# yosungho/LineTR

Measured on AMD Instinct MI355X. Metric: line_descriptors_per_sec, higher is better.
Workload: dtype f32 in/out; GEMMs as 6 bf16-split MFMA products, fp32 accumulate (fp32-faithful); 1 GPU; cfg3: 64 pairs/GPU of 640x480, 200 lines/image -> 199 sub-lines x 21 tokens, d_model=256, seeded weights; pairs_per_gpu=64, collective=none

## Files before the change

### experiments/csrc/lt_x_net.h

```cpp
#pragma once
#include "lt_gemm_sk.h"
#include "lt_gemm_st.h"
#include "lt_gemm_ro.h"
#include "lt_gemm_chain.h"
#include "lt_mlp_fused.h"
#include "lt_attn_st.h"
#include "lt_pairnet_host.h"

namespace {

int x_gemm(LinetrHandle* h, hipStream_t st, SplitGemmArgs& sa, const GemmW& w, int groups, const NormSpec* fused_norm,
           double fl, double by, bool& done) {
  const GemmArgs& g = sa.g;
  if (h->precision == LINETR_PREC_BF16X6 && LT_XENV("LINETR_GEMM_RO") != nullptr && groups == 1 && g.N % 256 == 0 && g.K % 32 == 0 &&
      w.st && g.lda % 4 == 0 && g.ldy % 4 == 0 && (!g.A2 || (g.lda2 % 4 == 0 && g.K1 % 16 == 0)) && (!g.R || g.ldr % 4 == 0) &&
      g.act != ACT_DIST && cdiv(g.M, 128) * (g.N / 256) >= 140) {
    RoGemmArgs a;
    a.A1 = g.A; a.lda1 = g.lda; a.nk1 = (g.A2 ? g.K1 : g.K) / 16; a.A2 = g.A2; a.lda2 = g.lda2; a.nk2 = g.A2 ? (g.K - g.K1) / 16 : 0;
    a.Wst = w.st; a.bias = g.bias ? g.bias : h->zeros; a.R = g.R; a.ldr = g.ldr; a.Y = g.Y; a.ldy = g.ldy;
    a.M = g.M; a.N = g.N; a.act = g.act;
    if (fused_norm) { a.norm = fused_norm->mode; a.gamma = fused_norm->gamma; a.beta = fused_norm->beta; a.add2 = fused_norm->add2; a.ldadd2 = D; a.eps = fused_norm->eps; }
    done = true;
    ProfScope ps(h, st, "gemm_bf16x6_ro128x256", fl, by);
    return gemm_ro_launch(a, st);
// ... 141 lines not shown
    if (int e = sig_mlp_fused_launch<2, 1>(a, st)) return e;
  } else {
    a.W1sp = S.W1.s3; a.W2sp = S.W2p.s3;
    ProfScope ps(h, st, "sig_mlp_bf16x6", fl, by);
    if (int e = sig_mlp_fused_launch<3, 0>(a, st)) return e;
  }
  LT_LAUNCH_CHECK();
  return 0;
}

int sig_network_fused_mlp(LinetrHandle* h, hipStream_t st, const TokenStage& ts, const int32_t* h_cu, const int* cu_dev, int n_images,
                          int N, int max_n, float* d_line_desc, FwdWs& w) {
  const LinetrModelConfig& c = h->cfg;
  const double attn_fl = attn_flops(h_cu, n_images);
  const int64_t sig_bn_off = 4 * (int64_t)(c.enc_channels[0] + c.enc_channels[1] + c.enc_channels[2] + c.enc_channels[3]);
  const int attn_kernel = sig_attn_plan(h, n_images, N, max_n).attn;
  const bool fused_qkv_attn = !LT_XENV("LINETR_NO_FUSED_QKV_ATTN") && h->precision == LINETR_PREC_BF16X6 && max_n <= 256 &&
                              (int64_t)n_images * HEADS >= 128;
  float *z = w.zA, *zn = w.zB;
  int e;
  for (size_t l = 0;; ++l) {
    const SigLayer& S = h->sig[l];
    if (fused_qkv_attn && S.Wqkv.st) {
      if ((e = sig_qkv_attention(h, st, S, z, cu_dev, n_images, N, attn_fl, w.msgp))) return e;
    } else {
      if ((e = run_gemm(h, st, S.Wqkv, N, {z, D}, {w.qkv, 3 * D}, ACT_NONE))) return e;
      if ((e = sig_attention(h, st, attn_kernel, w.qkv, 3 * D, cu_dev, n_images, N, max_n, attn_fl, w.msgp))) return e;
    }
    if (l + 1 == h->sig.size()) break;
    if ((e = run_sig_mlp(h, st, z, w.msgp, S, zn, N))) return e;
    std::swap(z, zn);
  }
  const size_t l = h->sig.size() - 1;
  if ((e = run_gemm(h, st, h->sig[l].W1, N, {z, D, w.msgp, D, D}, {w.hid, 2 * D}, ts.bn ? ACT_NONE : ACT_RELU))) return e;
  if (ts.bn && (e = bn_train_layer(st, *ts.bn, w.hid, N, 2 * D, 2 * D, h->bn_g[8 + l], h->bn_b[8 + l], sig_bn_off + (int64_t)l * 4 * D))) return e;
  NormSpec l2; l2.mode = 2;
  return run_gemm_norm(h, st, h->Wfin2, N, {z, D, w.hid, 2 * D, D}, nullptr, zn, d_line_desc, l2);
}

int sig_network_st(LinetrHandle* h, hipStream_t st, FwdWs& w, const XWs& x, const int32_t* h_cu, const int* cu_dev, int n_images,
                   int N, int max_n, float* d_line_desc) {
  auto gemm = [&](const char* role, const unsigned char* A1, int K1, const unsigned char* A2, int K2, const GemmW& W,
                  const unsigned char* R, unsigned char* Yst, float* Y, int act) -> int {
    const int Nout = W.rows;
    StGemmArgs a;
    a.A1 = A1; a.nk1 = K1 / 16; a.A2 = A2; a.nk2 = A2 ? K2 / 16 : 0;
    a.W = W.st; a.bias = W.b ? W.b : h->zeros; a.R = R; a.Yst = Yst; a.Y = Y; a.ldy = D; a.M = N; a.N = Nout; a.act = act;
// ... 114 lines not shown
```

### include/linetr_hip.h

```cpp
#ifndef LINETR_HIP_H
#define LINETR_HIP_H

#include <stdint.h>

#ifdef __cplusplus
extern "C" {
#endif

#define LINETR_ABI_VERSION 6

enum {
  LINETR_OK = 0,
  LINETR_E_ARG = -1,
  LINETR_E_HIP = -2,
  LINETR_E_WEIGHTS = -3,
  LINETR_E_ASSERT = -4,
  LINETR_E_WORKSPACE = -5,
  LINETR_E_CAPACITY = -6
};

typedef struct LinetrHandle LinetrHandle;

typedef struct {
  int32_t d_model;
// ... 437 lines not shown
int linetr_debug_posenc(LinetrHandle* h, int32_t which, const float* d_in0, const float* d_in1, const float* d_in2,
                           int64_t rows, float* d_out, void* stream);

int linetr_debug_gemm(LinetrHandle* h, const float* d_A, int32_t lda, const float* d_W, const float* d_bias,
                      const float* d_residual, float* d_Y, int32_t ldy, int32_t M, int32_t N, int32_t K,
                      int32_t act, int32_t cache_weights, void* stream);

#define LINETR_GEMM_TILE_WS 100
typedef struct {
  const float* A;   int32_t lda;
  const float* A2;  int32_t lda2;  int32_t K1;
  const float* W;
  const float* bias;
  const float* R;
  float* Y;         int32_t ldy;
  int32_t M, N, K, act;
  int32_t groups;   int64_t gA, gY;
  int32_t norm;     const float* gamma;  const float* beta;  const float* add2;  float eps;
  int32_t via_row_norm;
  int32_t tile;
} LinetrGemmCase;
int linetr_debug_gemm_case(LinetrHandle* h, const LinetrGemmCase* c, int32_t* tile_used, void* stream);

int linetr_debug_sig_attention(LinetrHandle* h, int32_t kernel, int32_t layer, const float* d_in, int32_t ld_in,
                               const int32_t* h_cu_sub, int32_t n_images, float* d_msg, int32_t* kernel_used, void* stream);

int linetr_debug_tok_mlp(LinetrHandle* h, int32_t variant, const float* d_pnt, const float* d_score, int64_t rows_word,
                         const float* d_sublines, const float* d_resp, const float* d_angle, int64_t rows_line,
                         float* d_out_word, float* d_out_line, int32_t max_blocks, int32_t* variant_used, void* stream);

int64_t linetr_debug_bn_train_workspace_bytes(const LinetrHandle* h, int32_t which, int64_t rows);
int linetr_debug_bn_train(LinetrHandle* h, int32_t which, float* d_z, int64_t rows, int32_t C, int32_t ld, const float* d_gamma,
                          const float* d_beta, const float* d_in0, const float* d_in1, const float* d_in2, float* d_out,
                          float momentum, float* d_running, float* d_batch, float* d_affine, int32_t* nb_used, void* d_ws,
                          int64_t ws_bytes, void* stream);

int linetr_debug_cls_pool(LinetrHandle* h, int32_t kernel, const LinetrLineRec* d_recs, int32_t K, const int32_t* d_sub2line,
                          int32_t N, int32_t T, const float* d_cpnt, const float* d_a4, int64_t first_pad, int32_t n_images,
                          const float* d_map, int32_t dense_is_nhwc, int32_t Hc, int32_t Wc, int32_t align_corners,
                          const float* d_desc_dense, float* d_pooled, int32_t* kernel_used, void* stream);

int linetr_debug_match(LinetrHandle* h, int32_t P, const int32_t* dims, const float* d_desc0, const int64_t* off_n0,
                       const int32_t* d_s2l0, const float* d_desc1, const int64_t* off_n1, const int32_t* d_s2l1, float thr,
                       int32_t mutual, float* d_dk, const int64_t* off_dk, int32_t* d_match01, const int64_t* off_k0, void* d_ws,
                       int64_t ws_bytes, int32_t path, int32_t seg1_global, int32_t cache_dk, int32_t device_table,
                       int32_t* path_used, void* stream);
// ... 53 lines not shown
```

### linetr_amd/csrc/linetr_net.hip

```cpp
#include <algorithm>
#include <array>
#include <numeric>
#include <set>

#include "lt_handle.h"
#include "lt_gemm.h"
#include "lt_gemm_split.h"
#include "lt_gemm_split16.h"
#include "lt_st_image.h"
#include "lt_gemm_small.h"
#include "lt_model.h"
#include "lt_attn.h"
#include "lt_attn_fused.h"
#include "lt_gemm_ws.h"
#include "lt_tokmlp.h"
#include "lt_token.h"
#include "lt_bntrain.h"

using namespace lt;

namespace {

const char* gemm_class_name(int precision, int tile, const GemmArgs& g, int groups) {
  static const auto names = [] {
// ... 597 lines not shown
}

int cls_pooling(LinetrHandle* h, hipStream_t& st, const TokenStage& ts, int n_images, int N, int T, FwdWs& w) {
  if (int e = cls_pool_launch(h, st, cls_pool_plan(ts.cpnt != nullptr, N), ts, n_images, N, T, w.act[ENC_WORD][3], w.pooled)) return e;
  return value_projection(h, st, N, w.pooled, w.att);
}

int sentence(LinetrHandle* h, hipStream_t& st, int N, FwdWs& w) {
  const LinetrModelConfig& c = h->cfg;
  int e;
  {
    NormSpec ns; ns.mode = 1; ns.gamma = h->ln1g; ns.beta = h->ln1b; ns.eps = 1e-6f;
    if ((e = run_gemm_norm(h, st, h->Wfc, N, {w.att, D}, nullptr, w.fc, w.o, ns))) return e;
  }
  if ((e = run_gemm(h, st, h->Wf1, N, {w.o, D}, {w.f1, c.d_inner}, ACT_GELU))) return e;
  NormSpec ns; ns.mode = 1; ns.gamma = h->ln2g; ns.beta = h->ln2b; ns.add2 = w.lpos; ns.eps = 1e-6f;
  return run_gemm_norm(h, st, h->Wf2, N, {w.f1, c.d_inner}, w.o, w.f2, w.zA, ns);
}

enum { SIGK_F32 = 0, SIGK_SMALL = 1, SIGK_SPLIT4 = 2, SIGK_SPLIT8 = 3, SIGK_FUSED = 4 };
struct SigAttnPlan {
  int attn;
  bool fold_next, fused;
  int kernel() const { return fused ? SIGK_FUSED : attn; }
};
SigAttnPlan sig_attn_plan(const LinetrHandle* h, int n_images, int N, int max_n) {
  SigAttnPlan p;
  const bool small_attn = h->precision != LINETR_PREC_F32 && (int64_t)n_images * HEADS * cdiv(max_n, 256) < 64;
  p.attn = h->precision == LINETR_PREC_F32 ? SIGK_F32 : small_attn ? SIGK_SMALL : max_n <= 128 ? SIGK_SPLIT4 : SIGK_SPLIT8;
  p.fold_next = small_attn && N <= SIG_FOLD_MAX_ROWS && !LT_XENV("LINETR_NO_SIG_FOLD");
  p.fused = !p.fold_next && !LT_XENV("LINETR_NO_FUSED_QKV_ATTN") && h->precision == LINETR_PREC_BF16X6 && max_n <= 256 &&
            (int64_t)n_images * HEADS >= 128;
  return p;
}

int sig_plan_servable(const LinetrHandle* h, const SigAttnPlan& p, int N, int max_n) {
  if (p.attn < SIGK_F32 || p.attn > SIGK_SPLIT8) return fail(LINETR_E_ARG, "sig plan: attention kernel %d outside 0 .. 3", p.attn);
  if (h->precision == LINETR_PREC_F32 && (p.attn != SIGK_F32 || p.fused))
    return fail(LINETR_E_ARG, "sig plan: the f32 mode runs sig_attn_kernel (0) only");
  if (p.fold_next) {
    if (p.fused) return fail(LINETR_E_ARG, "sig plan: fold_next and the fused projection + attention exclude each other");
    if (p.attn != SIGK_SMALL) return fail(LINETR_E_ARG, "sig plan: fold_next leaves q/k/v at row stride 1024, which sig_attn_small (1) alone reads");
    if (N > SIG_FOLD_MAX_ROWS) return fail(LINETR_E_ARG, "sig plan: fold_next has buffers for up to %d sub-lines (got %d)", SIG_FOLD_MAX_ROWS, N);
  }
  if (p.fused) {
    if (h->precision != LINETR_PREC_BF16X6) return fail(LINETR_E_ARG, "sig plan: the fused projection + attention runs in bf16x6 mode only");
// ... 3 lines not shown
  }
  return LINETR_OK;
}

int sig_attention(LinetrHandle* h, hipStream_t st, int kernel, const float* qkv, int ldq, const int* cu_dev, int n_images, int N,
                  int max_n, double fl, float* msg) {
  if (kernel == SIGK_F32) {
    ProfScope ps(h, st, "sig_attn", fl, (double)N * D * 16);
    hipLaunchKernelGGL(sig_attn_kernel, dim3(n_images, HEADS, cdiv(max_n, ATT_QT)), dim3(256), 0, st, qkv, cu_dev, msg);
  } else {
    ProfScope ps(h, st, "sig_attn_bf16x6", fl, (double)N * D * 16);
    if (kernel == SIGK_SMALL)
      hipLaunchKernelGGL(sig_attn_small_kernel, dim3(n_images, HEADS, cdiv(max_n, 32)), dim3(256), 0, st, qkv, cu_dev, msg, ldq);
    else if (kernel == SIGK_SPLIT4)
      hipLaunchKernelGGL(sig_attn_split_kernel<4>, dim3(n_images, HEADS, cdiv(max_n, ATT_QT)), dim3(256), 0, st, qkv, cu_dev, msg);
    else
      hipLaunchKernelGGL(sig_attn_split_kernel<8>, dim3(n_images, HEADS, cdiv(max_n, 256)), dim3(512), 0, st, qkv, cu_dev, msg);
  }
  LT_LAUNCH_CHECK();
  return LINETR_OK;
}

int sig_qkv_attention(LinetrHandle* h, hipStream_t st, const SigLayer& S, const float* z, const int* cu_dev, int n_images, int N,
                      double attn_fl, float* msg) {
  LT_HIP(allow_dynamic_lds<sig_qkv_attn_kernel>(FQA_LDS));
  ProfScope ps(h, st, "sig_qkv_attn_bf16x6", 2.0 * N * 3.0 * D * D + attn_fl, (double)N * D * 8);
  hipLaunchKernelGGL(sig_qkv_attn_kernel, dim3(n_images, HEADS), dim3(512), FQA_LDS, st, z, S.Wqkv.st, S.Wqkv.b,
                     cu_dev, msg);
  LT_LAUNCH_CHECK();
  return LINETR_OK;
}

int sig_network(LinetrHandle* h, hipStream_t& st, const TokenStage& ts, const int32_t* h_cu, const int* cu_dev, int n_images, int N,
                float* d_line_desc, FwdWs& w, const SigAttnPlan* forced = nullptr) {
  const LinetrModelConfig& c = h->cfg;
  int max_n = 0;
  for (int i = 0; i < n_images; ++i) max_n = std::max(max_n, h_cu[i + 1] - h_cu[i]);
  int e;
  const double attn_fl = attn_flops(h_cu, n_images);
  const int64_t sig_bn_off = 4 * (int64_t)(c.enc_channels[0] + c.enc_channels[1] + c.enc_channels[2] + c.enc_channels[3]);
  const SigAttnPlan plan = forced ? *forced : sig_attn_plan(h, n_images, N, max_n);
  const bool fold_next = plan.fold_next, fused_qkv_attn = plan.fused;
  float *z = w.zA, *zn = w.zB;
  int ldz = D;
  float *zq = w.zqA, *zq_next = w.zqB;
  const float* qkv = w.qkv;
  int ldq = 3 * D;
  for (size_t l = 0; l < h->sig.size(); ++l) {
    const SigLayer& S = h->sig[l];
    if (fused_qkv_attn && S.Wqkv.st) {
      if ((e = sig_qkv_attention(h, st, S, z, cu_dev, n_images, N, attn_fl, w.msgp))) return e;
    } else {
      if (!fold_next || l == 0)
        if ((e = run_gemm(h, st, S.Wqkv, N, {z, ldz}, {w.qkv, 3 * D}, ACT_NONE))) return e;
      if ((e = sig_attention(h, st, plan.attn, qkv, ldq, cu_dev, n_images, N, max_n, attn_fl, w.msgp))) return e;
    }
    if ((e = run_gemm(h, st, S.W1, N, {z, ldz, w.msgp, D, D}, {w.hid, 2 * D}, ts.bn ? ACT_NONE : ACT_RELU))) return e;
    if (ts.bn && (e = bn_train_layer(st, *ts.bn, w.hid, N, 2 * D, 2 * D, h->bn_g[8 + l], h->bn_b[8 + l], sig_bn_off + (int64_t)l * 4 * D))) return e;
    if (l + 1 == h->sig.size()) break;
    if (fold_next) {
      if ((e = run_gemm(h, st, S.Wnext, N, {z, ldz, w.hid, 2 * D, D}, {zq, 4 * D}, ACT_NONE))) return e;
      z = zq; ldz = 4 * D; qkv = zq + D; ldq = 4 * D;
      std::swap(zq, zq_next);
    } else {
      if ((e = run_gemm(h, st, S.W2, N, {w.hid, 2 * D}, {zn, D}, ACT_NONE, z))) return e;
      std::swap(z, zn);
    }
    if (w.tap)
      LT_HIP(hipMemcpy2DAsync(w.tap + (int64_t)l * N * D, D * sizeof(float), z, ldz * sizeof(float), D * sizeof(float), N,
                              hipMemcpyDeviceToDevice, st));
    if ((e = pipe_boundary(ts.pipe, CUT_SIG0 + (int)l, st))) return e;
  }
  NormSpec l2; l2.mode = 2;
  if (h->sig.empty()) return run_gemm_norm(h, st, h->Wfin, N, {z, D}, nullptr, zn, d_line_desc, l2);
// ... 349 lines not shown
  const int64_t tmp_at = bytes;
  if (c->norm && !fuse) bytes += (int64_t)M * D * sizeof(float);
  if (bytes > 0) LT_HIP(hipMalloc((void**)&buf, bytes));
  if (h->precision != LINETR_PREC_F32) split_copies(w, buf, at, true, st);
  int e = LINETR_OK;
  if (hipGetLastError() != hipSuccess) e = fail(LINETR_E_HIP, "debug_gemm_case: splitting the weights failed");
  force.launch = true;
  if (!e && c->norm && !fuse) {
    float* tmp = reinterpret_cast<float*>(buf + tmp_at);
    e = run_gemm(h, st, w, M, A, {tmp, D}, c->act, c->R, nullptr, nullptr, &force);
    if (!e) e = row_norm(h, st, tmp, M, ns, c->Y);
  } else if (!e) {
    e = run_gemm(h, st, w, M, A, {c->Y, c->ldy}, c->act, c->R, pg, fuse ? &ns : nullptr, &force);
  }
  (void)hipStreamSynchronize(st);
  if (buf) (void)hipFree(buf);
  return e;
}

extern "C" int linetr_debug_sig_attention(LinetrHandle* h, int32_t kernel, int32_t layer, const float* d_in, int32_t ld_in,
                                          const int32_t* h_cu, int32_t n_images, float* d_msg, int32_t* kernel_used, void* stream) {
  if (!h) return fail(LINETR_E_ARG, "debug_sig_attention: null handle");
  if (h->cfg.bn_batch_stats) return fail(LINETR_E_ARG, "debug_sig_attention: a training-mode handle (bn_batch_stats = 1) is not served");
  if (kernel < -1 || kernel > SIGK_FUSED) return fail(LINETR_E_ARG, "debug_sig_attention: kernel must be -1 .. 4");
  if (int e = check_cu(h_cu, n_images)) return e;
  const int N = h_cu[n_images];
  int max_n = 0;
  for (int i = 0; i < n_images; ++i) max_n = std::max(max_n, h_cu[i + 1] - h_cu[i]);
  const bool query_only = kernel == -1 && !d_in && !d_msg;
  if (kernel == -1) kernel = sig_attn_plan(h, n_images, N, max_n).kernel();
  if (kernel_used) *kernel_used = kernel;
  if (query_only) return LINETR_OK;
  if (kernel == SIGK_FUSED) {
    if (h->precision != LINETR_PREC_BF16X6) return fail(LINETR_E_ARG, "debug_sig_attention: the fused kernel runs in bf16x6 mode only");
    if (max_n > 256) return fail(LINETR_E_ARG, "debug_sig_attention: the fused kernel takes images of up to 256 sub-lines");
    if (layer < 0 || layer >= (int)h->sig.size()) return fail(LINETR_E_ARG, "debug_sig_attention: layer out of range");
    if (!h->sig[layer].Wqkv.st) return fail(LINETR_E_ARG, "debug_sig_attention: the layer has no split-tile weight image");
    if (ld_in != D) return fail(LINETR_E_ARG, "debug_sig_attention: the fused kernel reads z rows, ld_in must be 256");
  } else if (ld_in != 3 * D && !(kernel == SIGK_SMALL && ld_in == 4 * D)) {
    return fail(LINETR_E_ARG, "debug_sig_attention: ld_in must be 768 (or 1024, sig_attn_small only)");
  }
  if (N <= 0) return LINETR_OK;
  if (!d_in || !d_msg) return fail(LINETR_E_ARG, "debug_sig_attention: null tensor");
  if (((uintptr_t)d_in | (uintptr_t)d_msg) % 16) return fail(LINETR_E_ARG, "debug_sig_attention: tensors must be 16-byte aligned");
  LT_HIP(hipSetDevice(h->device));
  hipStream_t st = (hipStream_t)stream;
  int* cu_dev = nullptr;
  LT_HIP(hipMalloc((void**)&cu_dev, (n_images + 1) * sizeof(int)));
  int e = LINETR_OK;
  if (hipMemcpyAsync(cu_dev, h_cu, (n_images + 1) * sizeof(int), hipMemcpyHostToDevice, st) != hipSuccess)
    e = fail(LINETR_E_HIP, "debug_sig_attention: cu_sub upload failed");
  const double fl = attn_flops(h_cu, n_images);
  if (!e)
    e = kernel == SIGK_FUSED ? sig_qkv_attention(h, st, h->sig[layer], d_in, cu_dev, n_images, N, fl, d_msg)
                             : sig_attention(h, st, kernel, d_in, ld_in, cu_dev, n_images, N, max_n, fl, d_msg);
  (void)hipStreamSynchronize(st);
  (void)hipFree(cu_dev);
  return e;
}

extern "C" int linetr_debug_tok_mlp(LinetrHandle* h, int32_t variant, const float* d_pnt, const float* d_score, int64_t rows_word,
                                    const float* d_sublines, const float* d_resp, const float* d_angle, int64_t rows_line,
                                    float* d_out_word, float* d_out_line, int32_t max_blocks, int32_t* variant_used, void* stream) {
  if (!h) return fail(LINETR_E_ARG, "debug_tok_mlp: null handle");
  if (h->cfg.bn_batch_stats) return fail(LINETR_E_ARG, "debug_tok_mlp: a training-mode handle (bn_batch_stats = 1) is not served");
  if (variant < -1 || variant > TOKV_CHAIN) return fail(LINETR_E_ARG, "debug_tok_mlp: variant must be -1 .. 4");
  if (rows_word < 0 || rows_line < 0 || rows_word > INT32_MAX / 8 || rows_line > INT32_MAX / 8)
    return fail(LINETR_E_ARG, "debug_tok_mlp: row counts must be 0 .. %d", INT32_MAX / 8);
  if (max_blocks < 0) return fail(LINETR_E_ARG, "debug_tok_mlp: max_blocks must be 0 (one block per compute unit) or positive");
  if (!fused_mlp_enabled(h->cfg) || h->cfg.enc_channels[0] != 32 || h->cfg.enc_channels[3] != D)
    return fail(LINETR_E_ARG, "debug_tok_mlp: needs keyline_encoder [32,64,128,256]");
  const bool query_only = variant == -1 && !d_out_word && !d_out_line;
  bool word = rows_word > 0 && variant != TOKV_LINE, line = rows_line > 0 && variant != TOKV_WORD;
  if (variant == -1) {
    const TokMlpPlan plan = tok_mlp_plan(h, rows_word, rows_line);
    variant = plan.both >= 0 ? plan.both : (word && !plan.word) || (line && !plan.line) ? (int)TOKV_CHAIN : word ? (int)TOKV_WORD : line ? (int)TOKV_LINE : -1;
  }
// ... 161 lines not shown
  if (!e) e = cls_pool_launch(h, st, kernel, ts, n_images, N, T, d_a4, d_pooled);
  (void)hipStreamSynchronize(st);
  if (buf) (void)hipFree(buf);
  return e;
}

extern "C" int64_t linetr_debug_stage_workspace_bytes(const LinetrHandle* h, int32_t N, int32_t n_images) {
  if (!h || N < 0 || n_images < 0) return -1;
  return fwd_layout(h, std::max(N, 1), 0, std::max(n_images, 1), nullptr).total;
}

extern "C" int linetr_debug_stage(LinetrHandle* h, int32_t stage, int32_t N, const float* d_in0, const float* d_in1,
                                  const int32_t* h_cu, int32_t n_images, int32_t plan, float* d_out0, float* d_out1, float* d_out2,
                                  int32_t* plan_used, void* d_ws, int64_t ws_bytes, void* stream) {
  if (!h) return fail(LINETR_E_ARG, "debug_stage: null handle");
  if (h->cfg.bn_batch_stats) return fail(LINETR_E_ARG, "debug_stage: a training-mode handle (bn_batch_stats = 1) is not served");
  if (stage != LINETR_STAGE_TAIL && stage != LINETR_STAGE_SIG) return fail(LINETR_E_ARG, "debug_stage: stage must be 0 (tail) or 1 (sig)");
  if (N < 0 || N > INT32_MAX / (HEADS * POOLW)) return fail(LINETR_E_ARG, "debug_stage: row count must be 0 .. %d", INT32_MAX / (HEADS * POOLW));
  const bool sig = stage == LINETR_STAGE_SIG;
  SigAttnPlan p{};
  if (sig) {
    if (int e = check_cu(h_cu, n_images)) return e;
    if (h_cu[n_images] != N) return fail(LINETR_E_ARG, "debug_stage: cu_sub does not end at N");
    if (plan < -1 || (plan & ~LINETR_STAGE_FOLD_NEXT) > SIGK_FUSED)
      return fail(LINETR_E_ARG, "debug_stage: plan must be -1 or a kernel 0 .. 4 (+ %d: fold_next)", LINETR_STAGE_FOLD_NEXT);
    int max_n = 0;
    for (int i = 0; i < n_images; ++i) max_n = std::max(max_n, h_cu[i + 1] - h_cu[i]);
    p = sig_attn_plan(h, n_images, N, max_n);
    if (plan >= 0) {
      const int kernel = plan & ~LINETR_STAGE_FOLD_NEXT;
      p.fused = kernel == SIGK_FUSED;
      if (!p.fused) p.attn = kernel;
      p.fold_next = (plan & LINETR_STAGE_FOLD_NEXT) != 0;
      if (int e = sig_plan_servable(h, p, N, max_n)) return e;
    }
    if (plan_used) *plan_used = p.kernel() | (p.fold_next ? LINETR_STAGE_FOLD_NEXT : 0);
  } else if (plan != -1) {
    return fail(LINETR_E_ARG, "debug_stage: the tail has no plan to force (plan must be -1)");
  }
  if (N == 0) return LINETR_OK;
  if (!d_in0 || (!sig && !d_in1) || (sig && !d_out0) || !d_ws) return fail(LINETR_E_ARG, "debug_stage: null pointer");
  if (((uintptr_t)d_in0 | (uintptr_t)d_in1 | (uintptr_t)d_out0 | (uintptr_t)d_out1 | (uintptr_t)d_out2 | (uintptr_t)d_ws) % 16)
    return fail(LINETR_E_ARG, "debug_stage: tensors and the workspace must be 16-byte aligned");
  const int n_cu = sig ? n_images : 1;
  const int64_t ws_need = linetr_debug_stage_workspace_bytes(h, N, n_cu);
  if (ws_bytes < ws_need)
    return fail(LINETR_E_ARG, "debug_stage: workspace too small (%lld < %lld bytes)", (long long)ws_bytes, (long long)ws_need);
  LT_HIP(hipSetDevice(h->device));
  hipStream_t st = (hipStream_t)stream;
  FwdWs w = fwd_layout(h, N, 0, n_cu, (char*)d_ws);
  const size_t row_bytes = (size_t)N * D * sizeof(float);
  int e = LINETR_OK;
  auto copy = [&](float* dst, const float* src, size_t bytes) {
    if (!e && dst && hipMemcpyAsync(dst, src, bytes, hipMemcpyDeviceToDevice, st) != hipSuccess) e = fail(LINETR_E_HIP, "debug_stage: a device copy failed");
  };
  if (!sig) {
    w.lpos = const_cast<float*>(d_in1);
    e = value_projection(h, st, N, d_in0, w.att);
    if (!e) e = sentence(h, st, N, w);
// ... 12 lines not shown
```

### linetr_amd/csrc/lt_attn_fused.h

```cpp
#pragma once
#include "lt_st_image.h"
#include "lt_attn.h"

namespace lt {

constexpr int FQA_W_BYTES = 3 * 4 * ST_RB;
constexpr int FQA_SLOT = FQA_W_BYTES + 256 * 64;
constexpr int FQA_KEYS = 128;
constexpr int FQA_LDS = 4 * FQA_SLOT;

__global__ __launch_bounds__(512) void sig_qkv_attn_kernel(const float* __restrict__ z ,
                                                           const unsigned char* __restrict__ Wst ,
                                                           const float* __restrict__ bqkv ,
                                                           const int* __restrict__ cu_sub, float* __restrict__ out ) {
  extern __shared__ __attribute__((aligned(1024))) unsigned char fq_smem[];
  const int img = blockIdx.x, head = blockIdx.y;
  const int n0 = cu_sub[img], Ni = cu_sub[img + 1] - n0;
  if (Ni <= 0) return;
  const int tid = threadIdx.x, lane = tid & 63;
  const int wave = __builtin_amdgcn_readfirstlane(tid >> 6);
  const int h2 = lane >> 5, lq = lane & 31;
  const int q = wave * 32 + lq;
  const bool wave_active = wave * 32 < Ni;
  constexpr int RBW = 3 * D / 16, NK = D / 16;

  const int n_dma = wave < 2 ? 5 : 4;
  const unsigned lane16 = lane * 16;
  auto issue_one = [&](int d, int k, int slot) {
    const int x = wave + 8 * d;
    unsigned char* dst = fq_smem + slot * FQA_SLOT + x * 1024;
    if (x < 18) {
      const unsigned char* g = Wst + ((int64_t)k * RBW + (x / 6) * 16 + head * 4) * ST_RB + (x % 6) * 1024;
      LT_GLDS(g + lane16, dst, 0);
    } else {
      int row = (x - 18) * 16 + (lane >> 2);
      row = row < Ni ? row : Ni - 1;
      const float* g = z + (int64_t)(n0 + row) * D + k * 16 + (((lane & 3) - ((lane >> 4) & 3)) & 3) * 4;
      LT_GLDS(g, dst, 0);
    }
  };
  auto issue_step = [&](int k, int slot) {
#pragma unroll
    for (int d = 0; d < 5; ++d)
      if (d < n_dma) issue_one(d, k, slot);
  };
  auto wait_dma = [&](int steps) {
    if (steps <= 0) asm volatile("s_waitcnt vmcnt(0)" ::: "memory");
    else if (wave < 2) {
      if (steps == 1) asm volatile("s_waitcnt vmcnt(5)" ::: "memory");
      else asm volatile("s_waitcnt vmcnt(10)" ::: "memory");
    } else {
      if (steps == 1) asm volatile("s_waitcnt vmcnt(4)" ::: "memory");
      else asm volatile("s_waitcnt vmcnt(8)" ::: "memory");
    }
  };
#pragma unroll
  for (int k = 0; k < 4; ++k) issue_step(k, k);
  f32x16 acc[6];
  {
    const float* bp = bqkv + head * DH + 4 * h2;
#pragma unroll
    for (int i = 0; i < 6; ++i)
#pragma unroll
      for (int bq = 0; bq < 4; ++bq) {
        const f32x4 v = *reinterpret_cast<const f32x4*>(bp + (i >> 1) * D + (i & 1) * 32 + 8 * bq);
#pragma unroll
        for (int c = 0; c < 4; ++c) acc[i][4 * bq + c] = v[c];
      }
  }
  wait_dma(2);
  __builtin_amdgcn_s_barrier();
  asm volatile("" ::: "memory");

  const int lfrag = ((lane >> 4) & 1) * ST_RB + (lane >> 5) * 256 + (lane & 15) * 16;
  const int zrot = (lq >> 2) & 3;
  const int zoff0 = FQA_W_BYTES + (wave * 32 + lq) * 64 + ((2 * h2 + zrot) & 3) * 16;
  const int zoff1 = FQA_W_BYTES + (wave * 32 + lq) * 64 + ((2 * h2 + 1 + zrot) & 3) * 16;
  using Terms = split_terms<3>;
  auto read_w = [&](int k, int i, int p, bf16x8 (&wf)[3]) {
    wf[p] = *reinterpret_cast<const bf16x8*>(fq_smem + (k & 3) * FQA_SLOT + lfrag + ((i >> 1) * 4 + (i & 1) * 2) * ST_RB + p * ST_CHUNK);
  };
  auto split_z = [&](const f32x4& x0, const f32x4& x1, bf16x8 (&zf)[3]) {
    unsigned a[3], b[3], c[3], d[3];
    split_pair<3>(x0[0], x0[1], a); split_pair<3>(x0[2], x0[3], b);
    split_pair<3>(x1[0], x1[1], c); split_pair<3>(x1[2], x1[3], d);
#pragma unroll
    for (int p = 0; p < 3; ++p) {
      union { bf16x8 v; unsigned w[4]; } u;
      u.w[0] = a[p]; u.w[1] = b[p]; u.w[2] = c[p]; u.w[3] = d[p];
      zf[p] = u.v;
    }
  };
  bf16x8 zfA[3], zfB[3], wfA[3], wfB[3];
  {
    const f32x4 x0 = *reinterpret_cast<const f32x4*>(fq_smem + zoff0), x1 = *reinterpret_cast<const f32x4*>(fq_smem + zoff1);
    split_z(x0, x1, zfA);
#pragma unroll
    for (int p = 0; p < 3; ++p) read_w(0, 0, p, wfA);
  }
  auto step = [&](int s, bf16x8 (&zc)[3], bf16x8 (&zn)[3]) {
    f32x4 zr0, zr1;
    const bool more = s + 1 < NK;
#pragma unroll
    for (int m = 0; m < 36; ++m) {
      const int i = m / 6, t = m % 6;
      bf16x8 (&wc)[3] = (i & 1) ? wfB : wfA;
      bf16x8 (&wn)[3] = (i & 1) ? wfA : wfB;
      acc[i] = mfma_split<0>(wc[Terms::pa(t)], zc[Terms::pb(t)], acc[i]);
      if (t < 3) {
        if (i < 5) read_w(s, i + 1, t, wn);
        else read_w(s + 1, 0, t, wn);
      }
      if (m == 3) zr0 = *reinterpret_cast<const f32x4*>(fq_smem + ((s + 1) & 3) * FQA_SLOT + zoff0);
      if (m == 4) zr1 = *reinterpret_cast<const f32x4*>(fq_smem + ((s + 1) & 3) * FQA_SLOT + zoff1);
      if (m == 15) split_z(zr0, zr1, zn);
      if (m >= 18 && m < 23 && s >= 1 && s + 3 < NK) { if (m - 18 < n_dma) issue_one(m - 18, s + 3, (s + 3) & 3); }
      __builtin_amdgcn_sched_barrier(0);
    }
    asm volatile("s_waitcnt lgkmcnt(0)" ::: "memory");
    if (more) {
      wait_dma(s + 3 < NK ? 1 : 0);
      __builtin_amdgcn_s_barrier();
      asm volatile("" ::: "memory");
    }
    __builtin_amdgcn_sched_barrier(0);
  };
#pragma unroll 1
  for (int s = 0; s < NK; s += 2) {
    step(s, zfA, zfB);
    step(s + 1, zfB, zfA);
  }
  asm volatile("s_waitcnt vmcnt(0)" ::: "memory");

  auto pieces = [&](const f32x16& a, float scale, float (&v)[16]) {
#pragma unroll
    for (int r = 0; r < 16; ++r) v[r] = a[r] * scale;
#pragma unroll
    for (int c = 0; c < 4; ++c) { halves_swap(v[c], v[4 + c]); halves_swap(v[8 + c], v[12 + c]); }
  };
  auto split_run = [&](const float* x, bf16x8 (&o)[3]) {
    unsigned a[3], b[3], c[3], d[3];
    split_pair<3>(x[0], x[1], a); split_pair<3>(x[2], x[3], b);
    split_pair<3>(x[4], x[5], c); split_pair<3>(x[6], x[7], d);
#pragma unroll
    for (int p = 0; p < 3; ++p) {
      union { bf16x8 v; unsigned w[4]; } u;
      u.w[0] = a[p]; u.w[1] = b[p]; u.w[2] = c[p]; u.w[3] = d[p];
      o[p] = u.v;
    }
  };
  bf16x8 qf[4][3];
#pragma unroll
  for (int i = 0; i < 2; ++i) {
    float v[16];
    pieces(acc[i], LOG2E, v);
    split_run(v, qf[2 * i]);
    split_run(v + 8, qf[2 * i + 1]);
  }
  unsigned char* Ks = fq_smem;
  unsigned char* Vs = fq_smem + FQA_KEYS * ATS_RK;
  auto stage_kv = [&]() {
    const int r = (wave & 3) * 32 + lq;
#pragma unroll
    for (int i = 2; i < 6; ++i) {
      float v[16];
      pieces(acc[i], 1.f, v);
      unsigned char* dst = (i < 4 ? Ks + r * ATS_RK : Vs + r * ATS_RV) + ((i & 1) * 32 + 8 * h2) * 2;
#pragma unroll
      for (int g = 0; g < 2; ++g) {
        bf16x8 pl[3];
        split_run(v + 8 * g, pl);
#pragma unroll
        for (int p = 0; p < 3; ++p) *reinterpret_cast<bf16x8*>(dst + p * 128 + g * 32) = pl[p];
      }
    }
  };
  f32x16 o0, o1;
#pragma unroll
  for (int r = 0; r < 16; ++r) { o0[r] = 0.f; o1[r] = 0.f; }
  float m = -INFINITY, l = 0.f;
// ... 116 lines not shown
```

### linetr_amd/engine_debug.py

```python
from __future__ import annotations

import ctypes as C

import numpy as np
import torch

from . import _native as nat
from ._shapes import D, ptr


class _DebugSurface:
    def debug_posenc(self, which: str, in0, in1, in2=None):
        a, b = self._f32(in0), self._f32(in1)
        c = self._f32(in2) if in2 is not None else None
        rows = int(b.shape[0])
        out = torch.empty((rows, 128), dtype=torch.float32, device=self.device)
        self._call("linetr_debug_posenc", {"word": 0, "line": 1}[which], a.data_ptr(), b.data_ptr(), ptr(c), rows, out.data_ptr())
        return out

    def debug_gemm(self, A, W, bias=None, residual=None, act=0, cache_weights=False, out=None):
        W = self._f32(W)
        if A.dtype != torch.float32 or A.device != self.device or A.stride(1) != 1:
            A = self._f32(A)
        M, K = A.shape
# ... 66 lines not shown
            return t

        extent(A, M, K1, int(gA), "A")
        if A2 is not None:
            extent(A2, M, K - K1, int(gA), "A2")
        extent(out, M, N, gY, "out")
        if groups > 1 and gY < (M - 1) * out.stride(0) + N:
            raise ValueError("gY: the groups' outputs overlap")
        if residual is not None and extent(residual, M, N, 0, "residual").stride(0) != out.stride(0):
            raise ValueError("residual must share the output's row stride")
        vec = lambda t, n, what: None if t is None else extent(self._f32(t).reshape(1, -1), 1, n, 0, what)
        b, ga, be = vec(bias, groups * N, "bias"), vec(gamma, N, "gamma"), vec(beta, N, "beta")
        if add2 is not None and (extent(add2, M, N, 0, "add2").stride(0) != D or N != D):
            raise ValueError("add2 must have row stride 256")
        c = nat.GemmCase(A=ptr(A), lda=A.stride(0), A2=ptr(A2), lda2=A2.stride(0) if A2 is not None else 0, K1=K1 if A2 is not None else 0,
                         W=ptr(W), bias=ptr(b), R=ptr(residual), Y=ptr(out), ldy=out.stride(0), M=M, N=N, K=K, act=int(act),
                         groups=int(groups), gA=int(gA), gY=gY, norm=int(norm), gamma=ptr(ga), beta=ptr(be), add2=ptr(add2),
                         eps=float(eps), via_row_norm=int(bool(via_row_norm)), tile=self._gemm_tile_code(tile))
        used = C.c_int32(-1)
        self._call("linetr_debug_gemm_case", C.byref(c), C.byref(used))
        return (full if groups > 1 or full is out else out), self._gemm_tile_name(used.value)

    SIG_KERNELS = ("sig_attn", "sig_attn_small", "sig_attn_split4", "sig_attn_split8", "sig_qkv_attn")

    def sig_attention_kernel(self, cu_sub) -> int:
        cu = np.ascontiguousarray(np.asarray(cu_sub, dtype=np.int32))
        used = C.c_int32(-1)
        self._call("linetr_debug_sig_attention", -1, 0, None, 0, cu.ctypes.data, len(cu) - 1, None, C.byref(used))
        return used.value

    def debug_sig_attention(self, kernel, x, cu_sub, layer=0, out=None):
        if x.dtype != torch.float32 or x.device != self.device or x.stride(1) != 1:
            x = self._f32(x)
        cu = np.ascontiguousarray(np.asarray(cu_sub, dtype=np.int32))
        N = int(cu[-1]) if len(cu) else 0
        if int(x.shape[0]) < N:
            raise ValueError(f"{N} rows expected, got {int(x.shape[0])}")
        msg = out if out is not None else torch.empty((N, D), dtype=torch.float32, device=self.device)
        if msg.dtype != torch.float32 or msg.device != self.device or not msg.is_contiguous():
            raise ValueError("out must be a contiguous float32 tensor on the engine's device")
        used = C.c_int32(-1)
        self._call("linetr_debug_sig_attention", int(kernel), int(layer), x.data_ptr(), x.stride(0), cu.ctypes.data, len(cu) - 1, msg.data_ptr(),
                   C.byref(used))
        return msg, used.value

    TOK_MLP_VARIANTS = ("tok_mlp_word", "tok_mlp_line", "tok_mlp_dual", "tok_mlp_seq", "mlp123_gemm_chain")
# ... 160 lines not shown
```

Baseline: 10.49 million line-descriptors/s.

## Dedicate one wave as DMA producer in fused QKV-attention kernel

After: 10.70 million line-descriptors/s, median of 6. 2.0% higher.

```diff
diff --git a/experiments/csrc/lt_x_net.h b/experiments/csrc/lt_x_net.h
--- a/experiments/csrc/lt_x_net.h
+++ b/experiments/csrc/lt_x_net.h
@@ -187,7 +187,7 @@
   for (size_t l = 0;; ++l) {
     const SigLayer& S = h->sig[l];
     if (fused_qkv_attn && S.Wqkv.st) {
-      if ((e = sig_qkv_attention(h, st, S, z, cu_dev, n_images, N, attn_fl, w.msgp))) return e;
+      if ((e = sig_qkv_attention(h, st, S, z, cu_dev, n_images, N, max_n, false, attn_fl, w.msgp))) return e;
     } else {
       if ((e = run_gemm(h, st, S.Wqkv, N, {z, D}, {w.qkv, 3 * D}, ACT_NONE))) return e;
       if ((e = sig_attention(h, st, attn_kernel, w.qkv, 3 * D, cu_dev, n_images, N, max_n, attn_fl, w.msgp))) return e;
diff --git a/include/linetr_hip.h b/include/linetr_hip.h
--- a/include/linetr_hip.h
+++ b/include/linetr_hip.h
@@ -483,6 +483,7 @@
 } LinetrGemmCase;
 int linetr_debug_gemm_case(LinetrHandle* h, const LinetrGemmCase* c, int32_t* tile_used, void* stream);
 
+enum { LINETR_SIG_EIGHT_WAVES = 32 };
 int linetr_debug_sig_attention(LinetrHandle* h, int32_t kernel, int32_t layer, const float* d_in, int32_t ld_in,
                                const int32_t* h_cu_sub, int32_t n_images, float* d_msg, int32_t* kernel_used, void* stream);
 
diff --git a/linetr_amd/csrc/linetr_net.hip b/linetr_amd/csrc/linetr_net.hip
--- a/linetr_amd/csrc/linetr_net.hip
+++ b/linetr_amd/csrc/linetr_net.hip
@@ -643,6 +643,7 @@
 struct SigAttnPlan {
   int attn;
   bool fold_next, fused;
+  bool eight_waves = false;
   int kernel() const { return fused ? SIGK_FUSED : attn; }
 };
 SigAttnPlan sig_attn_plan(const LinetrHandle* h, int n_images, int N, int max_n) {
@@ -692,11 +693,12 @@
 }
 
 int sig_qkv_attention(LinetrHandle* h, hipStream_t st, const SigLayer& S, const float* z, const int* cu_dev, int n_images, int N,
-                      double attn_fl, float* msg) {
-  LT_HIP(allow_dynamic_lds<sig_qkv_attn_kernel>(FQA_LDS));
+                      int max_n, bool eight_waves, double attn_fl, float* msg) {
+  const bool producer = !eight_waves && max_n <= FQA_PRODUCER_ROWS;
+  LT_HIP(producer ? allow_dynamic_lds<sig_qkv_attn_kernel<true>>(FQA_LDS) : allow_dynamic_lds<sig_qkv_attn_kernel<false>>(FQA_LDS));
   ProfScope ps(h, st, "sig_qkv_attn_bf16x6", 2.0 * N * 3.0 * D * D + attn_fl, (double)N * D * 8);
-  hipLaunchKernelGGL(sig_qkv_attn_kernel, dim3(n_images, HEADS), dim3(512), FQA_LDS, st, z, S.Wqkv.st, S.Wqkv.b,
-                     cu_dev, msg);
+  hipLaunchKernelGGL(producer ? sig_qkv_attn_kernel<true> : sig_qkv_attn_kernel<false>, dim3(n_images, HEADS), dim3(512), FQA_LDS,
+                     st, z, S.Wqkv.st, S.Wqkv.b, cu_dev, msg);
   LT_LAUNCH_CHECK();
   return LINETR_OK;
 }
@@ -719,7 +721,7 @@
   for (size_t l = 0; l < h->sig.size(); ++l) {
     const SigLayer& S = h->sig[l];
     if (fused_qkv_attn && S.Wqkv.st) {
-      if ((e = sig_qkv_attention(h, st, S, z, cu_dev, n_images, N, attn_fl, w.msgp))) return e;
+      if ((e = sig_qkv_attention(h, st, S, z, cu_dev, n_images, N, max_n, plan.eight_waves, attn_fl, w.msgp))) return e;
     } else {
       if (!fold_next || l == 0)
         if ((e = run_gemm(h, st, S.Wqkv, N, {z, ldz}, {w.qkv, 3 * D}, ACT_NONE))) return e;
@@ -1115,14 +1117,17 @@
                                           const int32_t* h_cu, int32_t n_images, float* d_msg, int32_t* kernel_used, void* stream) {
   if (!h) return fail(LINETR_E_ARG, "debug_sig_attention: null handle");
   if (h->cfg.bn_batch_stats) return fail(LINETR_E_ARG, "debug_sig_attention: a training-mode handle (bn_batch_stats = 1) is not served");
-  if (kernel < -1 || kernel > SIGK_FUSED) return fail(LINETR_E_ARG, "debug_sig_attention: kernel must be -1 .. 4");
+  const bool eight_waves = kernel == (SIGK_FUSED | LINETR_SIG_EIGHT_WAVES);
+  if (eight_waves) kernel = SIGK_FUSED;
+  if (kernel < -1 || kernel > SIGK_FUSED)
+    return fail(LINETR_E_ARG, "debug_sig_attention: kernel must be -1 .. 4 (or 4 + %d: eight compute waves)", LINETR_SIG_EIGHT_WAVES);
   if (int e = check_cu(h_cu, n_images)) return e;
   const int N = h_cu[n_images];
   int max_n = 0;
   for (int i = 0; i < n_images; ++i) max_n = std::max(max_n, h_cu[i + 1] - h_cu[i]);
   const bool query_only = kernel == -1 && !d_in && !d_msg;
   if (kernel == -1) kernel = sig_attn_plan(h, n_images, N, max_n).kernel();
-  if (kernel_used) *kernel_used = kernel;
+  if (kernel_used) *kernel_used = kernel | (eight_waves ? LINETR_SIG_EIGHT_WAVES : 0);
   if (query_only) return LINETR_OK;
   if (kernel == SIGK_FUSED) {
     if (h->precision != LINETR_PREC_BF16X6) return fail(LINETR_E_ARG, "debug_sig_attention: the fused kernel runs in bf16x6 mode only");
@@ -1145,7 +1150,7 @@
     e = fail(LINETR_E_HIP, "debug_sig_attention: cu_sub upload failed");
   const double fl = attn_flops(h_cu, n_images);
   if (!e)
-    e = kernel == SIGK_FUSED ? sig_qkv_attention(h, st, h->sig[layer], d_in, cu_dev, n_images, N, fl, d_msg)
+    e = kernel == SIGK_FUSED ? sig_qkv_attention(h, st, h->sig[layer], d_in, cu_dev, n_images, N, max_n, eight_waves, fl, d_msg)
                              : sig_attention(h, st, kernel, d_in, ld_in, cu_dev, n_images, N, max_n, fl, d_msg);
   (void)hipStreamSynchronize(st);
   (void)hipFree(cu_dev);
@@ -1353,8 +1358,11 @@
   if (sig) {
     if (int e = check_cu(h_cu, n_images)) return e;
     if (h_cu[n_images] != N) return fail(LINETR_E_ARG, "debug_stage: cu_sub does not end at N");
+    const bool eight_waves = plan == (SIGK_FUSED | LINETR_SIG_EIGHT_WAVES);
+    if (eight_waves) plan = SIGK_FUSED;
     if (plan < -1 || (plan & ~LINETR_STAGE_FOLD_NEXT) > SIGK_FUSED)
-      return fail(LINETR_E_ARG, "debug_stage: plan must be -1 or a kernel 0 .. 4 (+ %d: fold_next)", LINETR_STAGE_FOLD_NEXT);
+      return fail(LINETR_E_ARG, "debug_stage: plan must be -1 or a kernel 0 .. 4 (+ %d: fold_next; 4 + %d: eight compute waves)",
+                  LINETR_STAGE_FOLD_NEXT, LINETR_SIG_EIGHT_WAVES);
     int max_n = 0;
     for (int i = 0; i < n_images; ++i) max_n = std::max(max_n, h_cu[i + 1] - h_cu[i]);
     p = sig_attn_plan(h, n_images, N, max_n);
@@ -1363,9 +1371,10 @@
       p.fused = kernel == SIGK_FUSED;
       if (!p.fused) p.attn = kernel;
       p.fold_next = (plan & LINETR_STAGE_FOLD_NEXT) != 0;
+      p.eight_waves = eight_waves;
       if (int e = sig_plan_servable(h, p, N, max_n)) return e;
     }
-    if (plan_used) *plan_used = p.kernel() | (p.fold_next ? LINETR_STAGE_FOLD_NEXT : 0);
+    if (plan_used) *plan_used = p.kernel() | (p.fold_next ? LINETR_STAGE_FOLD_NEXT : 0) | (p.eight_waves ? LINETR_SIG_EIGHT_WAVES : 0);
   } else if (plan != -1) {
     return fail(LINETR_E_ARG, "debug_stage: the tail has no plan to force (plan must be -1)");
   }
diff --git a/linetr_amd/csrc/lt_attn_fused.h b/linetr_amd/csrc/lt_attn_fused.h
--- a/linetr_amd/csrc/lt_attn_fused.h
+++ b/linetr_amd/csrc/lt_attn_fused.h
@@ -9,6 +9,10 @@
 constexpr int FQA_KEYS = 128;
 constexpr int FQA_LDS = 4 * FQA_SLOT;
 
+constexpr int FQA_PRODUCER_ROWS = 224;
+constexpr int FQA_PRODUCER_DMA = 18 + FQA_PRODUCER_ROWS / 16;
+
+template <bool PRODUCER>
 __global__ __launch_bounds__(512) void sig_qkv_attn_kernel(const float* __restrict__ z ,
                                                            const unsigned char* __restrict__ Wst ,
                                                            const float* __restrict__ bqkv ,
@@ -21,13 +25,13 @@
   const int wave = __builtin_amdgcn_readfirstlane(tid >> 6);
   const int h2 = lane >> 5, lq = lane & 31;
   const int q = wave * 32 + lq;
-  const bool wave_active = wave * 32 < Ni;
+  const bool producer = PRODUCER && wave == 7;
+  const bool wave_active = !producer && wave * 32 < Ni;
   constexpr int RBW = 3 * D / 16, NK = D / 16;
 
   const int n_dma = wave < 2 ? 5 : 4;
   const unsigned lane16 = lane * 16;
-  auto issue_one = [&](int d, int k, int slot) {
-    const int x = wave + 8 * d;
+  auto issue_piece = [&](int x, int k, int slot) {
     unsigned char* dst = fq_smem + slot * FQA_SLOT + x * 1024;
     if (x < 18) {
       const unsigned char* g = Wst + ((int64_t)k * RBW + (x / 6) * 16 + head * 4) * ST_RB + (x % 6) * 1024;
@@ -39,6 +43,7 @@
       LT_GLDS(g, dst, 0);
     }
   };
+  auto issue_one = [&](int d, int k, int slot) { issue_piece(wave + 8 * d, k, slot); };
   auto issue_step = [&](int k, int slot) {
 #pragma unroll
     for (int d = 0; d < 5; ++d)
@@ -54,84 +59,8 @@
       else asm volatile("s_waitcnt vmcnt(8)" ::: "memory");
     }
   };
-#pragma unroll
-  for (int k = 0; k < 4; ++k) issue_step(k, k);
   f32x16 acc[6];
-  {
-    const float* bp = bqkv + head * DH + 4 * h2;
-#pragma unroll
-    for (int i = 0; i < 6; ++i)
-#pragma unroll
-      for (int bq = 0; bq < 4; ++bq) {
-        const f32x4 v = *reinterpret_cast<const f32x4*>(bp + (i >> 1) * D + (i & 1) * 32 + 8 * bq);
-#pragma unroll
-        for (int c = 0; c < 4; ++c) acc[i][4 * bq + c] = v[c];
-      }
-  }
-  wait_dma(2);
-  __builtin_amdgcn_s_barrier();
-  asm volatile("" ::: "memory");
-
-  const int lfrag = ((lane >> 4) & 1) * ST_RB + (lane >> 5) * 256 + (lane & 15) * 16;
-  const int zrot = (lq >> 2) & 3;
-  const int zoff0 = FQA_W_BYTES + (wave * 32 + lq) * 64 + ((2 * h2 + zrot) & 3) * 16;
-  const int zoff1 = FQA_W_BYTES + (wave * 32 + lq) * 64 + ((2 * h2 + 1 + zrot) & 3) * 16;
-  using Terms = split_terms<3>;
-  auto read_w = [&](int k, int i, int p, bf16x8 (&wf)[3]) {
-    wf[p] = *reinterpret_cast<const bf16x8*>(fq_smem + (k & 3) * FQA_SLOT + lfrag + ((i >> 1) * 4 + (i & 1) * 2) * ST_RB + p * ST_CHUNK);
-  };
-  auto split_z = [&](const f32x4& x0, const f32x4& x1, bf16x8 (&zf)[3]) {
-    unsigned a[3], b[3], c[3], d[3];
-    split_pair<3>(x0[0], x0[1], a); split_pair<3>(x0[2], x0[3], b);
-    split_pair<3>(x1[0], x1[1], c); split_pair<3>(x1[2], x1[3], d);
-#pragma unroll
-    for (int p = 0; p < 3; ++p) {
-      union { bf16x8 v; unsigned w[4]; } u;
-      u.w[0] = a[p]; u.w[1] = b[p]; u.w[2] = c[p]; u.w[3] = d[p];
-      zf[p] = u.v;
-    }
-  };
-  bf16x8 zfA[3], zfB[3], wfA[3], wfB[3];
-  {
-    const f32x4 x0 = *reinterpret_cast<const f32x4*>(fq_smem + zoff0), x1 = *reinterpret_cast<const f32x4*>(fq_smem + zoff1);
-    split_z(x0, x1, zfA);
-#pragma unroll
-    for (int p = 0; p < 3; ++p) read_w(0, 0, p, wfA);
-  }
-  auto step = [&](int s, bf16x8 (&zc)[3], bf16x8 (&zn)[3]) {
-    f32x4 zr0, zr1;
-    const bool more = s + 1 < NK;
-#pragma unroll
-    for (int m = 0; m < 36; ++m) {
-      const int i = m / 6, t = m % 6;
-      bf16x8 (&wc)[3] = (i & 1) ? wfB : wfA;
-      bf16x8 (&wn)[3] = (i & 1) ? wfA : wfB;
-      acc[i] = mfma_split<0>(wc[Terms::pa(t)], zc[Terms::pb(t)], acc[i]);
-      if (t < 3) {
-        if (i < 5) read_w(s, i + 1, t, wn);
-        else read_w(s + 1, 0, t, wn);
-      }
-      if (m == 3) zr0 = *reinterpret_cast<const f32x4*>(fq_smem + ((s + 1) & 3) * FQA_SLOT + zoff0);
-      if (m == 4) zr1 = *reinterpret_cast<const f32x4*>(fq_smem + ((s + 1) & 3) * FQA_SLOT + zoff1);
-      if (m == 15) split_z(zr0, zr1, zn);
-      if (m >= 18 && m < 23 && s >= 1 && s + 3 < NK) { if (m - 18 < n_dma) issue_one(m - 18, s + 3, (s + 3) & 3); }
-      __builtin_amdgcn_sched_barrier(0);
-    }
-    asm volatile("s_waitcnt lgkmcnt(0)" ::: "memory");
-    if (more) {
-      wait_dma(s + 3 < NK ? 1 : 0);
-      __builtin_amdgcn_s_barrier();
-      asm volatile("" ::: "memory");
-    }
-    __builtin_amdgcn_sched_barrier(0);
-  };
-#pragma unroll 1
-  for (int s = 0; s < NK; s += 2) {
-    step(s, zfA, zfB);
-    step(s + 1, zfB, zfA);
-  }
-  asm volatile("s_waitcnt vmcnt(0)" ::: "memory");
-
+  bf16x8 qf[4][3];
   auto pieces = [&](const f32x16& a, float scale, float (&v)[16]) {
 #pragma unroll
     for (int r = 0; r < 16; ++r) v[r] = a[r] * scale;
@@ -149,13 +78,115 @@
       o[p] = u.v;
     }
   };
-  bf16x8 qf[4][3];
-#pragma unroll
-  for (int i = 0; i < 2; ++i) {
-    float v[16];
-    pieces(acc[i], LOG2E, v);
-    split_run(v, qf[2 * i]);
-    split_run(v + 8, qf[2 * i + 1]);
+  if (producer) {
+    static_assert(FQA_PRODUCER_DMA == 32, "the counted waits below say vmcnt(32)");
+    auto feed = [&](int k, int slot) {
+#pragma unroll
+      for (int x = 0; x < FQA_PRODUCER_DMA; ++x) issue_piece(x, k, slot);
+    };
+    feed(0, 0);
+    feed(1, 1);
+    feed(2, 2);
+    asm volatile("s_waitcnt vmcnt(32)" ::: "memory");
+    __builtin_amdgcn_s_barrier();
+    asm volatile("" ::: "memory");
+    feed(3, 3);
+#pragma unroll 1
+    for (int s = 0; s + 1 < NK; ++s) {
+      if (s >= 1 && s + 3 < NK) feed(s + 3, (s + 3) & 3);
+      if (s + 3 < NK) asm volatile("s_waitcnt vmcnt(32)" ::: "memory");
+      else asm volatile("s_waitcnt vmcnt(0)" ::: "memory");
+      __builtin_amdgcn_s_barrier();
+      asm volatile("" ::: "memory");
+    }
+  } else {
+    if constexpr (!PRODUCER) {
+#pragma unroll
+      for (int k = 0; k < 4; ++k) issue_step(k, k);
+    }
+    {
+      const float* bp = bqkv + head * DH + 4 * h2;
+#pragma unroll
+      for (int i = 0; i < 6; ++i)
+#pragma unroll
+        for (int bq = 0; bq < 4; ++bq) {
+          const f32x4 v = *reinterpret_cast<const f32x4*>(bp + (i >> 1) * D + (i & 1) * 32 + 8 * bq);
+#pragma unroll
+          for (int c = 0; c < 4; ++c) acc[i][4 * bq + c] = v[c];
+        }
+    }
+    if constexpr (!PRODUCER) wait_dma(2);
+    __builtin_amdgcn_s_barrier();
+    asm volatile("" ::: "memory");
+
+    const int lfrag = ((lane >> 4) & 1) * ST_RB + (lane >> 5) * 256 + (lane & 15) * 16;
+    const int zrot = (lq >> 2) & 3;
+    const int zoff0 = FQA_W_BYTES + (wave * 32 + lq) * 64 + ((2 * h2 + zrot) & 3) * 16;
+    const int zoff1 = FQA_W_BYTES + (wave * 32 + lq) * 64 + ((2 * h2 + 1 + zrot) & 3) * 16;
+    using Terms = split_terms<3>;
+    auto read_w = [&](int k, int i, int p, bf16x8 (&wf)[3]) {
+      wf[p] = *reinterpret_cast<const bf16x8*>(fq_smem + (k & 3) * FQA_SLOT + lfrag + ((i >> 1) * 4 + (i & 1) * 2) * ST_RB + p * ST_CHUNK);
+    };
+    auto split_z = [&](const f32x4& x0, const f32x4& x1, bf16x8 (&zf)[3]) {
+      unsigned a[3], b[3], c[3], d[3];
+      split_pair<3>(x0[0], x0[1], a); split_pair<3>(x0[2], x0[3], b);
+      split_pair<3>(x1[0], x1[1], c); split_pair<3>(x1[2], x1[3], d);
+#pragma unroll
+      for (int p = 0; p < 3; ++p) {
+        union { bf16x8 v; unsigned w[4]; } u;
+        u.w[0] = a[p]; u.w[1] = b[p]; u.w[2] = c[p]; u.w[3] = d[p];
+        zf[p] = u.v;
+      }
+    };
+    bf16x8 zfA[3], zfB[3], wfA[3], wfB[3];
+    {
+      const f32x4 x0 = *reinterpret_cast<const f32x4*>(fq_smem + zoff0), x1 = *reinterpret_cast<const f32x4*>(fq_smem + zoff1);
+      split_z(x0, x1, zfA);
+#pragma unroll
+      for (int p = 0; p < 3; ++p) read_w(0, 0, p, wfA);
+    }
+    auto step = [&](int s, bf16x8 (&zc)[3], bf16x8 (&zn)[3]) {
+      f32x4 zr0, zr1;
+      const bool more = s + 1 < NK;
+#pragma unroll
+      for (int m = 0; m < 36; ++m) {
+        const int i = m / 6, t = m % 6;
+        bf16x8 (&wc)[3] = (i & 1) ? wfB : wfA;
+        bf16x8 (&wn)[3] = (i & 1) ? wfA : wfB;
+        acc[i] = mfma_split<0>(wc[Terms::pa(t)], zc[Terms::pb(t)], acc[i]);
+        if (t < 3) {
+          if (i < 5) read_w(s, i + 1, t, wn);
+          else read_w(s + 1, 0, t, wn);
+        }
+        if (m == 3) zr0 = *reinterpret_cast<const f32x4*>(fq_smem + ((s + 1) & 3) * FQA_SLOT + zoff0);
+        if (m == 4) zr1 = *reinterpret_cast<const f32x4*>(fq_smem + ((s + 1) & 3) * FQA_SLOT + zoff1);
+        if (m == 15) split_z(zr0, zr1, zn);
+        if constexpr (!PRODUCER)
+          if (m >= 18 && m < 23 && s >= 1 && s + 3 < NK) { if (m - 18 < n_dma) issue_one(m - 18, s + 3, (s + 3) & 3); }
+        __builtin_amdgcn_sched_barrier(0);
+      }
+      asm volatile("s_waitcnt lgkmcnt(0)" ::: "memory");
+      if (more) {
+        if constexpr (!PRODUCER) wait_dma(s + 3 < NK ? 1 : 0);
+        __builtin_amdgcn_s_barrier();
+        asm volatile("" ::: "memory");
+      }
+      __builtin_amdgcn_sched_barrier(0);
+    };
+#pragma unroll 1
+    for (int s = 0; s < NK; s += 2) {
+      step(s, zfA, zfB);
+      step(s + 1, zfB, zfA);
+    }
+    asm volatile("s_waitcnt vmcnt(0)" ::: "memory");
+
+#pragma unroll
+    for (int i = 0; i < 2; ++i) {
+      float v[16];
+      pieces(acc[i], LOG2E, v);
+      split_run(v, qf[2 * i]);
+      split_run(v + 8, qf[2 * i + 1]);
+    }
   }
   unsigned char* Ks = fq_smem;
   unsigned char* Vs = fq_smem + FQA_KEYS * ATS_RK;
diff --git a/linetr_amd/engine_debug.py b/linetr_amd/engine_debug.py
--- a/linetr_amd/engine_debug.py
+++ b/linetr_amd/engine_debug.py
@@ -112,6 +112,7 @@
         return (full if groups > 1 or full is out else out), self._gemm_tile_name(used.value)
 
     SIG_KERNELS = ("sig_attn", "sig_attn_small", "sig_attn_split4", "sig_attn_split8", "sig_qkv_attn")
+    SIG_EIGHT_WAVES = 32
 
     def sig_attention_kernel(self, cu_sub) -> int:
         cu = np.ascontiguousarray(np.asarray(cu_sub, dtype=np.int32))
```
